# snayfach/MicrobeCensus

Hardware: AMD Instinct MI355X
Metric: reads/sec searched vs marker DB + AGS abs-error, 150 bp @ 1/2/4/8 GPU (higher is better)
Workload: dtype u8/int32

## Files before the change

microbecensus_amd/csrc/k_translate_seg.h:

```cpp
#pragma once
#include "mc_hip_common.h"

#define MC_TS_THREADS 64
#define MC_TS_WAVES (MC_TS_THREADS / 64)
#define MC_TS_READS (MC_TS_THREADS / 6)
#define MC_TS_NLNF(FP) ((FP) + 2 > 24 ? (FP) + 2 : 24)
#define MC_TS_STRIDE(FP) (((((FP) + 76 + 3) >> 2) | 1) << 2)
#define MC_TS_STAGE(L) ((((MC_TS_READS * (L)) > MC_TS_WAVES * 1488 ? (MC_TS_READS * (L)) : MC_TS_WAVES * 1488) + 15) & ~15)

struct McSegWaveLds { unsigned long long best[64]; uint32_t pre[66]; uint32_t pre2[66]; uint32_t bq[64]; uint16_t off[64]; uint8_t n[64]; };
static_assert(sizeof(McHsp) == 48 && sizeof(McGapTask) % 4 == 0, "k_eval_seeds copies its staging buffers as 16- and 4-byte words");
static_assert(sizeof(McSegWaveLds) == 1488, "MC_TS_STAGE reserves 1488 bytes per wave");
#ifdef MC_EXP_TIMING
__device__ unsigned long long g_ts_acc[12], g_ts_cnt[12];
#define MC_TS_TICK(k) do { const unsigned long long now_ = __builtin_readcyclecounter(); if (lane == 0) { ts_acc_[tcat_] += now_ - tlast_; ts_acc_[12 + tcat_] += 1; } tlast_ = now_; tcat_ = (k); } while (0)
#define MC_TS_BEGIN(k) __shared__ unsigned long long ts_acc_[24]; if (lane < 24) ts_acc_[lane] = 0; mc_wave_sync(); unsigned long long tlast_ = __builtin_readcyclecounter(); int tcat_ = (k)
#define MC_TS_PARAMS , unsigned long long &tlast_, int &tcat_, unsigned long long *ts_acc_
#define MC_TS_ARGS , tlast_, tcat_, ts_acc_
#define MC_TS_END do { mc_wave_sync(); if (lane < 12) { atomicAdd(&g_ts_acc[lane], ts_acc_[lane]); atomicAdd(&g_ts_cnt[lane], ts_acc_[12 + lane]); } } while (0)
#else
#define MC_TS_TICK(k) do { } while (0)
#define MC_TS_BEGIN(k) do { } while (0)
#define MC_TS_PARAMS
#define MC_TS_ARGS
#define MC_TS_END do { } while (0)
#endif
#define MC_SEG_KEY_ONE 0xBFF0000000000000ull

__device__ __forceinline__ unsigned long long mc_seg_key(double x)
{
    const unsigned long long u = (unsigned long long)__double_as_longlong(x);
    return (u >> 63) ? ~u : (u | 0x8000000000000000ull);
}

__device__ __forceinline__ void mc_seg_wave(const double *lnf, const int32_t *fx, const uint64_t *__restrict__ segtab, uint8_t *prot, int n, bool act, const McSegWS ws, McSegWaveLds *WL,
                                         const uint8_t *lds0, int lane MC_TS_PARAMS)
{
    const int W = (n <= 11) ? 8 : 12;
    MC_TS_TICK(0);
    enum { POP = 0, SCAN = 1, WAIT = 2, DONE = 3 };
    int st = (act && W <= n) ? POP : DONE;
    McBits192 Flo, Fhi, lo, nhi, mk;
    mc_bits_clear(Flo); mc_bits_clear(Fhi); mc_bits_clear(lo); mc_bits_clear(nhi); mc_bits_clear(mk);
    if (st != DONE) {
        mc_seg_window_flags_rg(fx, prot, n, W, Flo, Fhi);
        if (!(Flo.a | Flo.b | Flo.c)) st = DONE;
    }
    int sp = 1, base = 0, m = 0, i = 0, lowlim = 0, loi = 0, hii = 0;
    bool any = false;
    if (st != DONE) ws.stk[0] = (int16_t)(uint16_t)(n << 8);
    const unsigned long long ltmask = (1ull << lane) - 1;
    for (;;) {
        MC_TS_TICK(1);
        while (st == POP || st == SCAN) {
            if (st == POP) {
                if (sp == 0) { st = DONE; break; }
                sp--;
                base = MC_SEG_START(ws.stk[sp]); m = MC_SEG_LEN(ws.stk[sp]);
                if (W > m) continue;
                lo = mc_seg_flags_of(Flo, base, m, W);
                i = mc_bits_next(lo, 0);
                if (i >= m) continue;
                nhi = mc_bits_andnot(mc_bits_low(m), mc_seg_flags_of(Fhi, base, m, W));
                lowlim = 0; st = SCAN;
            }
            loi = mc_bits_prev(nhi, i) + 1; if (loi < lowlim) loi = lowlim;
            hii = mc_bits_next(nhi, i) - 1; if (hii > m - 1) hii = m - 1;
            st = WAIT;
        }
        const unsigned long long req = __ballot(st == WAIT);
        MC_TS_TICK(2);
        if (req == 0) break;
        const int nreq = __popcll(req);
        const int myr = __popcll(req & ltmask);
        const int myn = hii - loi + 1;
        if (st == WAIT) {
            WL->off[myr] = (uint16_t)((prot + base + loi) - lds0);
            WL->n[myr] = (uint8_t)myn;
            WL->best[myr] = MC_SEG_KEY_ONE; WL->bq[myr] = 0xFFFFFFFFu;
        }
        mc_wave_sync();
#define MC_SEG_CJ(j, sh) (((((j) >> (sh)) * (((j) >> (sh)) + 1)) << (sh)) / 2 + ((j) & ((1 << (sh)) - 1)) * (((j) >> (sh)) + 1))
        int sh0 = 3, sh1 = 3;
        {
            int K = 0, j0 = 0;
            if (lane < nreq) { const int nn = WL->n[lane], minlen = (nn - 100 > 1) ? nn - 100 : 1; K = nn - minlen; j0 = nn - 15 > 0 ? (nn - 15 < K ? nn - 15 : K) : 0; }
            uint32_t s0 = 0, s1 = 0;
#pragma unroll
            for (int sh = 2; sh >= 0; sh--) {
                const uint32_t c1 = (uint32_t)MC_SEG_CJ(j0, sh), c0 = (uint32_t)MC_SEG_CJ(K, sh) - c1;
                const uint32_t t0 = (uint32_t)__builtin_amdgcn_readlane((int)mc_wave_scan_add(c0), 63), t1 = (uint32_t)__builtin_amdgcn_readlane((int)mc_wave_scan_add(c1), 63);
                if (t0 <= 64) sh0 = sh;
                if (t1 <= 64) sh1 = sh;
            }
            {
                const uint32_t c1 = sh1 == 0 ? (uint32_t)MC_SEG_CJ(j0, 0) : sh1 == 1 ? (uint32_t)MC_SEG_CJ(j0, 1) : sh1 == 2 ? (uint32_t)MC_SEG_CJ(j0, 2) : (uint32_t)MC_SEG_CJ(j0, 3);
// ... 67 lines not shown
                        if (w0 == wlast) break;
                        mc_seg_shift(ws.comp, ws.sv, s[w0], s[w0 + len]);
                    }
                }
            }
            MC_TS_TICK(5);
            const bool cand = ok && key < MC_SEG_KEY_ONE;
            const unsigned long long old = WL->best[r];
            mc_wave_sync();
            if (cand) atomicMin(&WL->best[r], key);
            mc_wave_sync();
            const unsigned long long nb = WL->best[r];
            if (ok && nb != old) WL->bq[r] = 0xFFFFFFFFu;
            mc_wave_sync();
            if (cand && key == nb) atomicMin(&WL->bq[r], kq);
            mc_wave_sync();
        }
        }
#undef MC_SEG_CJ
        MC_TS_TICK(6);
        if (st == WAIT) {
            const uint32_t q = WL->bq[myr];
            int lend = 0, rend = myn - 1;
            if (q != 0xFFFFFFFFu) {
                int j = (int)((sqrtf((float)(8u * q + 1u)) - 1.0f) * 0.5f);
                while ((uint32_t)((j + 1) * (j + 2) / 2) <= q) j++;
                while ((uint32_t)(j * (j + 1) / 2) > q) j--;
                const int len = myn - j, w0 = (int)q - j * (j + 1) / 2;
                lend = w0; rend = len + w0 - 1;
            }
            const int leftend = loi + lend, rightend = hii - (myn - rend - 1);
            if (i < leftend) {
                const int l2 = loi, r2 = leftend - 1;
                sp = mc_seg_push(ws.stk, sp, W, base + l2, r2 - l2 + 1);
            }
            mk = mc_bits_or(mk, mc_bits_range(base + leftend, base + rightend));
            any = true;
            lowlim = ((hii < rightend) ? hii : rightend) + 1;
            i = mc_bits_next(lo, lowlim);
            st = i < m ? SCAN : POP;
        }
        mc_wave_sync();
    }
    MC_TS_TICK(7);
    if (any) for (int k = 0; k < n; k++) if (mc_bits_test(mk, k)) prot[k] = MC_INV;
    MC_TS_TICK(10);
}

__device__ __forceinline__ int mc_translate_frame_lds(const uint8_t *cod, const uint8_t *read, int len, int frame, uint8_t *prot)
{
    const int o = frame % 3;
    int n = (len - o) / 3;
    if (n < 0) n = 0;
    const bool rc = frame >= 3;
    const uint32_t set = rc ? MC_NT_RC_SET : MC_NT_FWD_SET, perm = rc ? MC_NT_RC_PERM : MC_NT_FWD_PERM;
    const uint8_t *p = read + (rc ? len - 1 - o : o);
    const int s = rc ? -1 : 1;
    int i = 0;
    for (; i + 8 <= n; i += 8) {
        uint32_t b[24], w[2] = {0, 0};
#pragma unroll
        for (int k = 0; k < 24; k++) b[k] = p[s * (3 * i + k)];
#pragma unroll
        for (int k = 0; k < 8; k++) {
            const int a0 = mc_nt_code(b[3 * k], set, perm), a1 = mc_nt_code(b[3 * k + 1], set, perm), a2 = mc_nt_code(b[3 * k + 2], set, perm);
            const uint32_t aa = cod[(16 * a0 + 4 * a1 + a2) & 63];
            w[k >> 2] |= ((a0 | a1 | a2) < 0 ? (uint32_t)MC_INV : aa) << (8 * (k & 3));
        }
        *(uint32_t *)(prot + i) = w[0];
        *(uint32_t *)(prot + i + 4) = w[1];
    }
    for (; i < n; i++) {
        const int a0 = mc_nt_code(p[s * (3 * i)], set, perm), a1 = mc_nt_code(p[s * (3 * i + 1)], set, perm), a2 = mc_nt_code(p[s * (3 * i + 2)], set, perm);
        const uint8_t aa = cod[(16 * a0 + 4 * a1 + a2) & 63];
        prot[i] = (a0 | a1 | a2) < 0 ? (uint8_t)MC_INV : aa;
    }
    return n;
}

template <bool STAGED>
__global__ void __attribute__((amdgpu_waves_per_eu(4, 4))) __launch_bounds__(MC_TS_THREADS) k_translate_seg(const McTables *__restrict__ T, const uint8_t *__restrict__ reads, int L,
                                                       int64_t nreads, uint8_t *__restrict__ frames, int FP, const uint64_t *__restrict__ segtab)
{
    extern __shared__ __attribute__((aligned(16))) uint8_t smem[];
    const int tid = threadIdx.x;
    const int64_t r0 = (int64_t)blockIdx.x * MC_TS_READS;
    const int nr = (int)((nreads - r0) < MC_TS_READS ? (nreads - r0) : MC_TS_READS);
    const int rbytes = nr * L;
    const int stride = MC_TS_STRIDE(FP);
    __shared__ int32_t fxs[64];
#ifdef MC_EXP_TIMING
    const int lane = mc_lane();
#endif
    MC_TS_BEGIN(8);
    uint8_t *sreads = smem;
    const int nlnf = MC_TS_NLNF(FP);
    double *lnf = (double *)(smem + (STAGED ? MC_TS_STAGE(L) : MC_TS_STAGE(0)));
    uint8_t *rows = (uint8_t *)(lnf + nlnf);
    __shared__ __attribute__((aligned(4))) uint8_t cod[64];
    if (tid < 64) fxs[tid] = T->seg_dout[tid];
    if (tid < 16) ((uint32_t *)cod)[tid] = ((const uint32_t *)T->codon)[tid];
    for (int i = tid; i < nlnf; i += MC_TS_THREADS) lnf[i] = T->lnfac[i];
    if (STAGED) {
        const uint8_t *src = reads + r0 * L;
        const int head = (int)((4 - ((uintptr_t)src & 3)) & 3), nhead = head < rbytes ? head : rbytes;
        if (tid < nhead) sreads[tid] = src[tid];
        const int nw = (rbytes - nhead) >> 2;
        if (nhead == 0) for (int i = tid; i < nw; i += MC_TS_THREADS) ((uint32_t *)sreads)[i] = ((const uint32_t *)src)[i];
        else for (int i = tid; i < nw; i += MC_TS_THREADS) { const uint32_t w = ((const uint32_t *)(src + nhead))[i]; uint8_t *d = sreads + nhead + 4 * i; d[0] = (uint8_t)w; d[1] = (uint8_t)(w >> 8); d[2] = (uint8_t)(w >> 16); d[3] = (uint8_t)(w >> 24); }
        for (int i = nhead + 4 * nw + tid; i < rbytes; i += MC_TS_THREADS) sreads[i] = src[i];
    }
    __syncthreads();
    MC_TS_TICK(9);
    const int lr = tid / 6, f = tid - lr * 6;
    uint8_t *prot = rows + (size_t)tid * stride;
    int n = 0;
    if (lr < nr) n = mc_translate_frame_lds(cod, STAGED ? sreads + lr * L : reads + (r0 + lr) * L, L, f, prot);
    __syncthreads();
    {
        McSegWS ws; ws.comp = prot + FP; ws.sv = prot + FP + 20; ws.stk = (int16_t *)(prot + FP + 44);
        mc_seg_wave(lnf, fxs, segtab, prot, n, lr < nr, ws, (McSegWaveLds *)smem + (tid >> 6), rows, mc_lane() MC_TS_ARGS);
        if (lr < nr) for (int i = n; i < FP; i++) prot[i] = MC_INV;
    }
    __syncthreads();
    {
        uint32_t *dst = (uint32_t *)(frames + r0 * 6 * FP);
        const int total = nr * 6 * FP / 4, fpw = FP / 4;
        for (int i = tid; i < total; i += MC_TS_THREADS) { const int row = i / fpw, col = i - row * fpw; dst[i] = *(const uint32_t *)(rows + (size_t)row * stride + 4 * col); }
    }
    MC_TS_TICK(0);
    MC_TS_END;
}
```

microbecensus_amd/csrc/mc_core.h:

```cpp
#pragma once
#include <stdint.h>

#if defined(__HIPCC__)
#include <hip/hip_runtime.h>
#define MC_HD __host__ __device__ __forceinline__
#define MC_HDN __host__ __device__
#else
#define MC_HD inline
#define MC_HDN inline
struct uint4 { uint32_t x, y, z, w; };
inline uint4 make_uint4(uint32_t x, uint32_t y, uint32_t z, uint32_t w) { uint4 v; v.x = x; v.y = y; v.z = z; v.w = w; return v; }
#endif

#define MC_NBUCKET 1000000
#define MC_INV 20
#define MC_INVGRP 10
#define MC_MAXAA 170
#define MC_SMAX 4096
#define MC_MAX_M8 500
#define MC_LNFAC_N 400

#define MC_GAP_OPEN 11
#define MC_GAP_EXT 1
#define MC_SEG_FXBITS 24
// ... 176 lines not shown
    }
    double ans2 = lnfac[total];
    for (int i = 0; sv[i] != 0; i++) ans2 = ans2 - lnfac[sv[i]];
    double t = (double)total * 2.995732273553991;
    return (ans2 + ans1) - t;
}
MC_HD void mc_seg_trim(const McTables &T, const uint8_t *s, int n, int *leftend, int *rightend)
{
    int lend = 0, rend = n - 1, minlen = 1;
    double minprob = 1.0;
    uint8_t comp[20], sv[21];
    if (n - 100 > minlen) minlen = n - 100;
    for (int len = n; len > minlen; len--) {
        mc_seg_comp(s, len, comp);
        for (int i = 0;; i++) {
            mc_seg_state(comp, sv);
            double prob = mc_seg_getprob(T.lnfac, sv, len);
            if (prob < minprob) { minprob = prob; lend = i; rend = len + i - 1; }
            if (i + 1 + len > n) break;
            if (s[i] < 20) comp[s[i]]--;
            if (s[i + len] < 20) comp[s[i + len]]++;
        }
    }
    *leftend = *leftend + lend;
    *rightend = *rightend - (n - rend - 1);
}
#define MC_SEG_STK 16
static_assert(MC_MAXAA / 13 < MC_SEG_STK && MC_MAXAA <= 255, "the SEG work list: n / (W + 1) entries of 8 + 8 bits");
#ifndef MC_SEG_ON_FULL
#define MC_SEG_ON_FULL() ((void)0)
#endif
#define MC_SEG_START(e) ((int)((uint16_t)(e) & 255))
#define MC_SEG_LEN(e) ((int)((uint16_t)(e) >> 8))
MC_HD int mc_seg_push(int16_t *stk, int sp, int W, int start, int len)
{
    if (len < W) return sp;
    if (sp >= MC_SEG_STK) { MC_SEG_ON_FULL(); return sp; }
    stk[sp] = (int16_t)(uint16_t)(start | (len << 8));
    return sp + 1;
}
MC_HDN void mc_seg_mask(const McTables &T, const uint8_t *prot, int n, uint8_t *maskbits , double *H)
{
    int W = (n <= 11) ? 8 : 12;
    int16_t stk[MC_SEG_STK];
    int sp = 0;
    for (int i = 0; i < (MC_MAXAA + 7) / 8; i++) maskbits[i] = 0;
    stk[0] = (int16_t)(uint16_t)(n << 8); sp = 1;
    while (sp > 0) {
        sp--;
        int base = MC_SEG_START(stk[sp]), m = MC_SEG_LEN(stk[sp]);
        const uint8_t *s = prot + base;
        if (W > m) continue;
        {
            uint8_t comp[20], sv[21];
            int start = 0;
            mc_seg_comp(s, W, comp);
            mc_seg_state(comp, sv);
            double ent = mc_seg_entropy(T, W, sv);
            for (int i = 0; i <= m - 1; i++) {
                H[i] = ent;
                if (start + 1 + W <= m) {
                    if (s[start] < 20) comp[s[start]]--;
                    if (s[start + W] < 20) comp[s[start + W]]++;
                    start++;
                    mc_seg_state(comp, sv);
                    ent = mc_seg_entropy(T, W, sv);
                }
            }
        }
        int last = m - 1, lowlim = 0;
        for (int i = 0; i <= last; i++) {
            if (H[i] <= 2.2 && H[i] != -1.0) {
                int j, loi, hii, leftend, rightend;
// ... 143 lines not shown
    uint32_t x = (lo ^ (hi << 7) ^ (((hi >> 28) * 0x924000u) & 0x04444000u)) * 0xBA1BF32Fu;
    x ^= x >> 15;
    h1 = x >> (32 - MC_SEGTAB_LOG2);
    h2 = (x >> 6) & (MC_SEGTAB_SLOTS - 1);
}
MC_HD uint64_t mc_segtab_lookup(const uint64_t *tab, uint64_t hist, int len)
{
    const uint64_t k = hist | ((uint64_t)len << 60);
    uint32_t h1, h2;
    mc_segtab_slots(k, h1, h2);
    if (tab[2 * h1] == k) return tab[2 * h1 + 1];
    return tab[2 * h2] == k ? tab[2 * h2 + 1] : 0;
}

MC_HD void mc_seg_trim_rg(const double *lnfac, const uint8_t *s, int n, int *leftend, int *rightend)
{
    int lend = 0, rend = n - 1;
    double minprob = 1.0;
    McRgState st0; st0.clo = 0; st0.chi = 0; st0.sv = 0;
    for (int k = 0; k < n; k++) mc_rg_add(st0, s[k]);
    for (int len = n; len > 1; len--) {
        McRgState st = st0;
        for (int i = 0;; i++) {
            const double prob = mc_rg_getprob(lnfac, st.sv, len);
            if (prob < minprob) { minprob = prob; lend = i; rend = len + i - 1; }
            if (i + 1 + len > n) break;
            mc_rg_remove(st, s[i]); mc_rg_add(st, s[i + len]);
        }
        mc_rg_remove(st0, s[len - 1]);
    }
    *leftend = *leftend + lend;
    *rightend = *rightend - (n - rend - 1);
}
struct McBits192 { uint64_t a, b, c; };
MC_HD void mc_bits_clear(McBits192 &x) { x.a = 0; x.b = 0; x.c = 0; }
MC_HD void mc_bits_set(McBits192 &x, int i) { uint64_t m = 1ull << (i & 63); if (i < 64) x.a |= m; else if (i < 128) x.b |= m; else x.c |= m; }
MC_HD bool mc_bits_test(const McBits192 &x, int i) { uint64_t w = (i < 64) ? x.a : (i < 128) ? x.b : x.c; return (w >> (i & 63)) & 1; }

MC_HDN void mc_seg_mask_ws(const McTables &T, uint8_t *prot, int n, const McSegWS &ws)
{
    int W = (n <= 11) ? 8 : 12;
    McBits192 lo, hi, mk;
    mc_bits_clear(mk);
    if (W > n) return;
    int sp = 1;
    ws.stk[0] = (int16_t)(uint16_t)(n << 8);
    bool any = false;
    while (sp > 0) {
        sp--;
        int base = MC_SEG_START(ws.stk[sp]), m = MC_SEG_LEN(ws.stk[sp]);
        const uint8_t *s = prot + base;
        if (W > m) continue;
        mc_bits_clear(lo); mc_bits_clear(hi);
        {
            int start = 0;
            bool anylo = false;
            mc_seg_comp(s, W, ws.comp);
            mc_seg_state(ws.comp, ws.sv);
            double ent = mc_seg_entropy(T, W, ws.sv);
            for (int i = 0; i <= m - 1; i++) {
                if (ent <= 2.2) { mc_bits_set(lo, i); anylo = true; }
                if (ent <= 2.5) mc_bits_set(hi, i);
                if (start + 1 + W <= m) {
                    mc_seg_shift(ws.comp, ws.sv, s[start], s[start + W]);
                    start++;
                    ent = mc_seg_entropy(T, W, ws.sv);
                }
            }
            if (!anylo) continue;
        }
// ... 91 lines not shown
    else { r.a = w0; r.b = w1; r.c = w2; }
    return r;
}
MC_HD McBits192 mc_bits_low(int n)
{
    McBits192 r;
    r.a = n >= 64 ? ~0ull : (n > 0 ? (1ull << n) - 1 : 0);
    r.b = n >= 128 ? ~0ull : (n > 64 ? (1ull << (n - 64)) - 1 : 0);
    r.c = n >= 192 ? ~0ull : (n > 128 ? (1ull << (n - 128)) - 1 : 0);
    return r;
}
MC_HD McBits192 mc_bits_and(const McBits192 &x, const McBits192 &y) { McBits192 r; r.a = x.a & y.a; r.b = x.b & y.b; r.c = x.c & y.c; return r; }
MC_HD McBits192 mc_bits_or(const McBits192 &x, const McBits192 &y) { McBits192 r; r.a = x.a | y.a; r.b = x.b | y.b; r.c = x.c | y.c; return r; }
MC_HD McBits192 mc_bits_andnot(const McBits192 &x, const McBits192 &y) { McBits192 r; r.a = x.a & ~y.a; r.b = x.b & ~y.b; r.c = x.c & ~y.c; return r; }
MC_HD McBits192 mc_bits_range(int lo, int hi) { return mc_bits_andnot(mc_bits_low(hi + 1), mc_bits_low(lo)); }
MC_HD int mc_bits_next(const McBits192 &x, int from)
{
    if (from >= 192) return 192;
    McBits192 y = mc_bits_andnot(x, mc_bits_low(from));
    if (y.a) return __builtin_ctzll(y.a);
    if (y.b) return 64 + __builtin_ctzll(y.b);
    if (y.c) return 128 + __builtin_ctzll(y.c);
    return 192;
}
MC_HD int mc_bits_prev(const McBits192 &x, int from)
{
    if (from < 0) return -1;
    McBits192 y = mc_bits_and(x, mc_bits_low(from + 1));
    if (y.c) return 191 - __builtin_clzll(y.c);
    if (y.b) return 127 - __builtin_clzll(y.b);
    if (y.a) return 63 - __builtin_clzll(y.a);
    return -1;
}
MC_HD McBits192 mc_seg_flags_of(const McBits192 &F, int base, int m, int W)
{
    McBits192 r = mc_bits_and(mc_bits_shr(F, base), mc_bits_low(m - W + 1));
    if (mc_bits_test(r, m - W)) r = mc_bits_or(r, mc_bits_range(m - W + 1, m - 1));
    return r;
}
MC_HD void mc_seg_window_flags(const int32_t *fx, const uint8_t *s, int n, int W, uint8_t *comp, McBits192 &Flo, McBits192 &Fhi)
{
    mc_bits_clear(Flo); mc_bits_clear(Fhi);
    int S = 0, t = 0;
    for (int i = 0; i < 20; i++) comp[i] = 0;
    for (int i = 0; i < W; i++) { const int r = s[i]; if (r < 20) { const int c = comp[r]; S += fx[16 + c]; comp[r] = (uint8_t)(c + 1); t++; } }
    for (int x = 0;; x++) {
        if (S >= fx[32 + t]) mc_bits_set(Flo, x);
        if (S >= fx[48 + t]) mc_bits_set(Fhi, x);
        if (x + 1 + W > n) break;
        const int o = s[x], e = s[x + W];
        if (o < 20) { const int c = comp[o]; S += fx[c]; comp[o] = (uint8_t)(c - 1); t--; }
        if (e < 20) { const int c = comp[e]; S += fx[16 + c]; comp[e] = (uint8_t)(c + 1); t++; }
    }
}
MC_HD void mc_seg_window_flags_rg(const int32_t *fx, const uint8_t *s, int n, int W, McBits192 &Flo, McBits192 &Fhi)
{
    uint64_t clo = 0; uint32_t chi = 0;
    int S = 0, t = 0;
    for (int i = 0; i < W; i++) {
        const int r = s[i];
        if (r < 20) {
            const int sh = (r & 15) * 4;
            const int c = (r < 16) ? (int)((clo >> sh) & 15) : (int)((chi >> sh) & 15);
            S += fx[16 + c]; t++;
            if (r < 16) clo += 1ull << sh; else chi += 1u << sh;
        }
    }
    const int nwin = n - W + 1;
    uint64_t wl[3] = {0, 0, 0}, wh[3] = {0, 0, 0};
#if defined(__HIP_DEVICE_COMPILE__)
#pragma unroll
#endif
    for (int q = 0; q < 3; q++) {
        uint64_t a = 0, b = 0;
        const int x1 = nwin - 64 * q < 64 ? nwin - 64 * q : 64;
        for (int xx = 0; xx < x1; xx++) {
            const int x = 64 * q + xx;
            a |= (uint64_t)(S >= fx[32 + t]) << xx;
            b |= (uint64_t)(S >= fx[48 + t]) << xx;
            if (x + 1 < nwin) {
                const int o = s[x], e = s[x + W];
                if (o < 20) {
                    const int sh = (o & 15) * 4;
                    const int c = (o < 16) ? (int)((clo >> sh) & 15) : (int)((chi >> sh) & 15);
                    S += fx[c]; t--;
                    if (o < 16) clo -= 1ull << sh; else chi -= 1u << sh;
                }
                if (e < 20) {
                    const int sh = (e & 15) * 4;
                    const int c = (e < 16) ? (int)((clo >> sh) & 15) : (int)((chi >> sh) & 15);
                    S += fx[16 + c]; t++;
                    if (e < 16) clo += 1ull << sh; else chi += 1u << sh;
                }
            }
        }
        wl[q] = a; wh[q] = b;
    }
    Flo.a = wl[0]; Flo.b = wl[1]; Flo.c = wl[2];
    Fhi.a = wh[0]; Fhi.b = wh[1]; Fhi.c = wh[2];
}
MC_HDN void mc_seg_mask_fx2(const double *lnfac, const int32_t *fx, uint8_t *prot, int n, const McSegWS &ws)
{
    const int W = (n <= 11) ? 8 : 12;
    if (W > n) return;
    McBits192 Flo, Fhi, mk;
    mc_bits_clear(mk);
    mc_seg_window_flags(fx, prot, n, W, ws.comp, Flo, Fhi);
    if (!(Flo.a | Flo.b | Flo.c)) return;
    int sp = 1;
    ws.stk[0] = (int16_t)(uint16_t)(n << 8);
    bool any = false;
    while (sp > 0) {
        sp--;
        const int base = MC_SEG_START(ws.stk[sp]), m = MC_SEG_LEN(ws.stk[sp]);
        const uint8_t *s = prot + base;
        if (W > m) continue;
        const McBits192 lo = mc_seg_flags_of(Flo, base, m, W), hi = mc_seg_flags_of(Fhi, base, m, W);
        const McBits192 nhi = mc_bits_andnot(mc_bits_low(m), hi);
        int lowlim = 0;
        for (int i = mc_bits_next(lo, 0); i < m; i = mc_bits_next(lo, i + 1)) {
            int loi = mc_bits_prev(nhi, i) + 1; if (loi < lowlim) loi = lowlim;
            int hii = mc_bits_next(nhi, i) - 1; if (hii > m - 1) hii = m - 1;
            int leftend = loi, rightend = hii;
            if (rightend - leftend + 1 <= 15) mc_seg_trim_rg(lnfac, s + leftend, rightend - leftend + 1, &leftend, &rightend);
            else mc_seg_trim_ws(lnfac, s + leftend, rightend - leftend + 1, &leftend, &rightend, ws);
            if (i < leftend) {
                const int lend = loi, rend = leftend - 1;
                sp = mc_seg_push(ws.stk, sp, W, base + lend, rend - lend + 1);
            }
            mk = mc_bits_or(mk, mc_bits_range(base + leftend, base + rightend));
            any = true;
            i = (hii < rightend) ? hii : rightend;
            lowlim = i + 1;
        }
    }
    if (any) for (int i = 0; i < n; i++) if (mc_bits_test(mk, i)) prot[i] = MC_INV;
}

MC_HD int mc_klen(uint32_t k)
{
    int low = (k & 0xf) != 0xf;
    int l = ((k & 0xff) != 0xff) ? 3 + low : 2 + low;
    l -= ((k & 0xfff) == 0xfff);
    l -= (k == 0xffff);
    return l;
}
MC_HD bool mc_key_lb_less(uint32_t dbk, uint32_t qk)
{
    int ld = mc_klen(dbk), lq = mc_klen(qk), n = ld < lq ? ld : lq;
    if (n != 0) { int sh = (4 - n) * 4; int a = (int)(dbk >> sh), b = (int)(qk >> sh); if (a != b) return a < b; }
    return ld < lq;
}
MC_HD bool mc_key_ub_less(uint32_t qk, uint32_t dbk)
{
    int ld = mc_klen(dbk), lq = mc_klen(qk), n = lq <= ld ? lq : ld;
    if (n == 0) return lq < ld;
    int sh = (4 - n) * 4; int a = (int)(qk >> sh), b = (int)(dbk >> sh);
    if (a == b) return false;
    return a < b;
}
struct McSeedCount { uint32_t lookups, keyprobes, tasks; };

MC_HD int mc_key_range(const McIndex &X, int seed, uint32_t qk, int *nst_out, McSeedCount *sc)
// ... 658 lines not shown
```

microbecensus_amd/csrc/mc_hip.hip:

```cpp
#include "mc_hip_common.h"
#include "k_translate_seg.h"
#include "k_enumerate.h"
#include "k_eval_seeds.h"
#include "k_gapped.h"
#include "k_order.h"
#include "k_finish.h"
#include "mc_stages.h"
#include "k_grid.h"
#include "k_simulate.h"
#include "k_community.h"
#include "k_varlen.h"
#include "k_classes.h"
#include "k_bootstrap.h"
#include "k_wfit.h"
#include "mc_pieces.h"
#include "mc_ahead.h"
#include "mc_owned.h"
#include "mc_abund.h"

#include <map>

struct McCtx {
    McStream stream; hipStream_t side = nullptr, side2 = nullptr;
    McEvent ev[8], ev_fork, ev_join, ev_join2;
    McEvent ev_wait[2]; bool waited = false;
    int64_t cap_reads = 0; int pool_len = 0;
    int ts_staged = -1;
    uint32_t cap_tasks = 0, cap_gaps = 0, cap_hsps = 0, cap_rows = 0;
    McDev<uint8_t> d_frames_base[2]; uint8_t *d_frames = nullptr;
    uint8_t *frames_of(int b) const { return d_frames_base[b] + 64; }
    void frames_use(int b) { d_frames = frames_of(b); }
    McDev<unsigned long long> d_stats;
    McDev<McSeedTask> d_tasks; McDev<McGapTask> d_gaps; McDev<McHsp> d_hsps, d_v, d_tmp;
    McDev<uint64_t> d_k64, d_hkeys, d_hplace, d_places; McDev<uint32_t> d_idx, d_idxo, d_heads, d_scan, d_gsz, d_nv, d_ghist;
    McDev<uint32_t> d_counters;
    McDev<McRow> d_rows; McDev<uint32_t> d_nrow, d_rowoff; McDev<McBestHit> d_best, d_bestof; McDev<uint8_t> d_low, d_cand;
    McDev<McGapCell> d_gws_full; McDev<uint32_t> d_retry, d_retry2;
    McDev<unsigned long long> d_gtab; uint32_t gtab_slots = 0; McDev<uint32_t> d_gleader; McDev<McFlankOut> d_fout;
    McPin<uint32_t> h_c; McPin<unsigned long long> h_stats; McPin<McBestHit> h_best; size_t h_best_cap = 0;
    const uint8_t *reads = nullptr; int64_t n = 0, first_read_id = 0, first = 0;
    int ahead_from = -1;
    bool predicts = false;
    bool own_a0 = true;
    uint32_t ntasks = 0, ngaps = 0, gpad = 0, nh = 0, nh_all = 0, nheads = 0, nrows = 0, nbest = 0, nsegs = 0;
    bool busy = false;
};

struct mc_handle {
    McHostIndex H;
    std::vector<int32_t> fam;
    int nfam = 0, device = 0;
    McDev<uint8_t> d_res_base; uint8_t *d_res = nullptr; McDev<uint32_t> d_off, d_bstart, d_post; McDev<unsigned long long> d_post8; McDev<uint16_t> d_keys; McDev<int32_t> d_fam;
    McDev<McTables> d_T; McDev<McClassPars> d_P;
    McTables hT; McClassPars hP;
    int read_len = 0, FP = 0; bool run_set = false;
    McDev<uint32_t> d_bitmap;
    McDev<McBucketRec> d_rec;
    McDev<uint32_t> d_filt, d_wild, d_pair; McDev<uint64_t> d_segtab; McDev<unsigned long long> d_rt;
    bool fast_enum = false;
    bool count_traffic = false;
// ... 456 lines not shown
            for (int k = 0; k < 7; k++) fprintf(stderr, "ev-timing %-21s total %9.1f Mcycles (lane 0 of every wave)\n", en[k], ev[k] / 1e6);
            unsigned long long z8[8] = {0, 0, 0, 0, 0, 0, 0, 0};
            HIPCK(hipMemcpyToSymbol(HIP_SYMBOL(g_ev_acc), z8, sizeof z8));
            unsigned long long tr[4];
            HIPCK(hipMemcpyFromSymbol(tr, HIP_SYMBOL(g_ev_turns), sizeof tr));
            fprintf(stderr, "ev-turns forward: %.1f M lane-turns in %.2f M wave-turns = %.1f lanes of 64; backward: %.1f M in %.2f M = %.1f lanes\n", tr[0] / 1e6, tr[1] / 1e6, tr[1] ? (double)tr[0] / (double)tr[1] : 0.0,
                    tr[2] / 1e6, tr[3] / 1e6, tr[3] ? (double)tr[2] / (double)tr[3] : 0.0);
            HIPCK(hipMemcpyToSymbol(HIP_SYMBOL(g_ev_turns), z8, sizeof tr));
        }
        const char *nm[8] = {"group starts", "groups", "scan, items", "sort", "threshold, ranks", "heap sort", "rows", "other"};
        for (int k = 0; k < 8; k++) fprintf(stderr, "fh-timing %-17s total %9.1f Mcycles %9llu entries\n", nm[k], acc[k] / 1e6, cnt[k]);
        {
            unsigned long long w[12];
            HIPCK(hipMemcpyFromSymbol(w, HIP_SYMBOL(g_fh_worst), sizeof w));
            fprintf(stderr, "fh-worst read: %llu stacked HSPs, %.3f Mcycles:", w[0] & 0xFFFFF, (double)(w[0] >> 20) / 1e6);
            for (int k = 0; k < 8; k++) fprintf(stderr, " %s %.3f", nm[k], (double)w[1 + k] / 1e6);
            fprintf(stderr, "\n");
            unsigned long long z12[12] = {0, 0, 0, 0, 0, 0, 0, 0, 0, 0, 0, 0};
            HIPCK(hipMemcpyToSymbol(HIP_SYMBOL(g_fh_worst), z12, sizeof z12));
        }
        unsigned long long z[8] = {0, 0, 0, 0, 0, 0, 0, 0};
        HIPCK(hipMemcpyToSymbol(HIP_SYMBOL(g_fh_acc), z, sizeof z)); HIPCK(hipMemcpyToSymbol(HIP_SYMBOL(g_fh_cnt), z, sizeof z));
    }
    return 0;
}
#else
static int exp_timing_dump(mc_handle *, McCtx &, char) { return 0; }
#endif

static int stage_a0(mc_handle *h, McCtx &c, hipStream_t st, const uint8_t *reads, uint8_t *into, int64_t at, int64_t n, hipEvent_t e0, hipEvent_t e1)
{
    uint8_t *frames = into + at * 6 * h->FP;
    HIPCK(hipEventRecord(e0, st));
    if (mc_translate_launch(h->d_T, h->d_segtab, reads, h->read_len, h->FP, n, frames, st, &c.ts_staged)) return -1;
    HIPCK(hipEventRecord(e1, st));
    return 0;
}

static int stage_a(mc_handle *h, McCtx &c, int64_t covered)
{
    const int64_t n = c.n;
    hipStream_t st = c.stream;
    c.ntasks = c.ngaps = c.gpad = c.nh = c.nheads = c.nrows = c.nbest = c.nsegs = 0;
    HIPCK(hipMemsetAsync(c.d_counters, 0, sizeof(uint32_t) * C_N, st));
    HIPCK(hipMemsetAsync(c.d_stats, 0, sizeof(unsigned long long) * S_N, st));
    if (h->best_only) HIPCK(hipMemsetAsync(c.d_cand, 0, (size_t)n, st));
    HIPCK(hipMemsetAsync(c.d_low, 0, (size_t)n, st));
    c.own_a0 = covered < n;
    if (!c.own_a0) HIPCK(hipEventRecord(c.ev[1], st));
    else if (stage_a0(h, c, st, c.reads + covered * h->read_len, c.d_frames, covered, n - covered, c.ev[0], c.ev[1])) return -1;
    if (exp_timing_dump(h, c, 'a')) return -1;
    const McRun R = run_of(h);
    const McSeedBufs B = carve_seed(h, c);
    const McSeedKernel kind = !h->fast_enum ? MC_SEED_PLAIN : h->count_traffic ? MC_SEED_COUNTING : MC_SEED_QUEUES;
    if (mc_enumerate_launch(R, B, n, kind, st)) return -1;
    HIPCK(hipEventRecord(c.ev[2], st));
    if (mc_eval_seeds_launch(R, B, kind == MC_SEED_QUEUES, st)) return -1;
    HIPCK(hipEventRecord(c.ev[3], st));
    return counters_to_host(c);
}

static int stage_b(mc_handle *h, McCtx &c)
{
    hipStream_t st = c.stream;
    if (c.h_c[C_OVERFLOW]) { g_err = "seed task / HSP / gap task buffer overflow"; return -2; }
    c.ntasks = c.h_c[C_TASKS];
    const uint32_t ngaps = c.ngaps = c.h_c[C_GAPS];
// ... 213 lines not shown
    return range_end(h, c);
}

static int range_begin_checked(mc_handle *h, int64_t first, int64_t count, int64_t first_read_id, bool predicts)
{
    if (range_check(h, first, count)) return -1;
    if (count <= 0) { g_err = "mc_range_begin: an empty range"; return -1; }
    if (h->pipe_nout) { g_err = "mc_range_begin: a range is in flight already (mc_range_end first)"; return -1; }
    const int rc = range_begin(h, h->ctx, first, count, first_read_id, predicts);
    if (rc) return rc;
    h->pipe_nout = 1;
    return 0;
}
extern "C" int mc_range_begin(mc_handle *h, int64_t first, int64_t count, int64_t first_read_id) { return range_begin_checked(h, first, count, first_read_id, true); }

static int range_end_next(mc_handle *h, int64_t first, int64_t count) { return range_end(h, h->ctx, first, count); }

extern "C" int64_t mc_ranges_translated_ahead(const mc_handle *h) { return h ? h->ahead_used : 0; }
extern "C" float mc_ahead_kernel_ms(const mc_handle *h) { return h ? h->ahead_ms : 0.0f; }

extern "C" int mc_range_end(mc_handle *h)
{
    if (!h) { g_err = "null handle"; return -1; }
    if (h->pipe_nout == 0) { g_err = "mc_range_end: no range in flight"; return -1; }
    HIPCK(hipSetDevice(h->device));
    h->pipe_nout = 0;
    return range_end(h, h->ctx);
}

extern "C" int mc_ranges_in_flight(const mc_handle *h) { return h ? h->pipe_nout : 0; }

extern "C" int64_t mc_debug_stage(mc_handle *h, int what, void *dst, int64_t cap_bytes, int32_t *record_bytes)
{
    if (!h || !h->run_set || what < 0 || what > 5) { g_err = "mc_debug_stage: bad argument"; return -1; }
    if (h->pipe_nout) { g_err = "mc_debug_stage: ranges are in flight"; return -1; }
    HIPCK(hipSetDevice(h->device));
    ahead_drop(h);
    const McCtx &c = h->ctx;
    if (what == 4) {
        if (!c.h_c) { g_err = "mc_debug_stage: no range has run"; return -1; }
        const uint32_t v[3] = {c.h_c[C_ITEMS], c.h_c[C_RETRY], c.h_c[C_RETRY2]};
        if (record_bytes) *record_bytes = (int32_t)sizeof(uint32_t);
        if (dst && (int64_t)sizeof v <= cap_bytes) memcpy(dst, v, sizeof v);
        return (int64_t)sizeof v;
    }
    if (what == 5) {
        if (c.ts_staged < 0) { g_err = "mc_debug_stage: no range has run"; return -1; }
        const uint32_t v = (uint32_t)c.ts_staged;
        if (record_bytes) *record_bytes = (int32_t)sizeof v;
        if (dst && (int64_t)sizeof v <= cap_bytes) memcpy(dst, &v, sizeof v);
        return (int64_t)sizeof v;
    }
    const void *src = nullptr; int64_t bytes = 0; int32_t rec = 0;
    if (what == 0) { src = c.d_frames; rec = h->FP; bytes = c.n * 6 * (int64_t)h->FP; }
    else if (what == 1) { src = c.d_tasks; rec = (int32_t)sizeof(McSeedTask); bytes = (int64_t)c.ntasks * rec; }
    else if (what == 2) { src = c.d_gaps; rec = (int32_t)sizeof(McGapTask); bytes = (int64_t)c.ngaps * rec; }
    else { src = c.d_hsps; rec = (int32_t)sizeof(McHsp); bytes = (int64_t)(c.nh_all + (c.h_c ? c.h_c[C_HPAD] : 0u)) * rec; }
    if (record_bytes) *record_bytes = rec;
    if (dst && bytes && bytes <= cap_bytes) { HIPCK(hipStreamSynchronize(c.stream)); HIPCK(hipMemcpy(dst, src, (size_t)bytes, hipMemcpyDeviceToHost)); }
    return bytes;
}

extern "C" int mc_set_counting(mc_handle *h, int on)
{
    if (!h) { g_err = "null handle"; return -1; }
    ahead_drop(h);
    h->count_traffic = on != 0;
    return 0;
}

extern "C" int mc_run(mc_handle *h, int64_t first_read_id) { return h ? mc_run_range(h, 0, h->nreads, first_read_id) : -1; }

#define MC_STREAM_BATCH 2000000
static int64_t stream_batch()
{
    if (const char *e = getenv("MC_STREAM_BATCH")) { const long long v = atoll(e); if (v >= 1000 && v <= MC_STREAM_BATCH) return (int64_t)v; }
    return MC_STREAM_BATCH;
}
struct McBatchSlot { uint8_t *pin = nullptr, *dev = nullptr; int64_t n = 0, first = 0; int state = 0;  int64_t rc = 0; };

static int run_stream(mc_handle *h, const std::function<int64_t(uint8_t *, int64_t, int64_t *)> &fetch, int64_t first_read_id, int64_t expect_reads = 0)
// ... 1659 lines not shown
```

microbecensus_amd/csrc/mc_stages.h:

```cpp
#pragma once
#include "k_translate_seg.h"
#include "k_enumerate.h"
#include "k_eval_seeds.h"
#include "k_gapped.h"
#include "k_order.h"
#include "k_finish.h"

static constexpr uint32_t MC_CUS = 256u;
static constexpr int MC_GAP_THREADS_FULL = 16 * 1024;
static constexpr uint32_t MC_GAP_SORT_BLOCKS = 512u;
static constexpr uint32_t MC_GAP_GRID_MAX = MC_CUS * 8u;
static constexpr uint32_t MC_GAP_GRID2 = MC_CUS * 4u;
static constexpr uint32_t MC_GAP_GRID_FULL = (uint32_t)MC_GAP_THREADS_FULL / 128u;
static constexpr uint32_t MC_BIN_BLOCKS = MC_CUS * 8u;
static inline size_t mc_order_heavy_lds(uint32_t cap) { return (size_t)cap * 18; }
static inline size_t mc_finish_heavy_lds(int maxn) { return (size_t)maxn * 16 + 3 * (size_t)(maxn + 2) * 2; }
static inline size_t mc_heap_lanes_lds() { return (size_t)(MC_MAX_M8 + 2) * 64 * 4; }
static inline size_t mc_finish_lds(int tpb, int items) { return (size_t)tpb * (items * 16 + 16); }

struct McRun { const McTables *T; McIndex X; const McClassPars *P; const int32_t *fam; int L, FP; };
struct McFork { hipStream_t side, side2; hipEvent_t fork, join, join2; };

static int mc_translate_launch(const McTables *T, const uint64_t *segtab, const uint8_t *reads, int L, int FP, int64_t n, uint8_t *frames, hipStream_t st, int *staged_out = nullptr)
{
    const size_t lds_rest = (size_t)MC_TS_NLNF(FP) * 8 + (size_t)MC_TS_THREADS * MC_TS_STRIDE(FP);
    const size_t lds_staged = (size_t)MC_TS_STAGE(L) + lds_rest, lds_direct = (size_t)MC_TS_STAGE(0) + lds_rest;
    static const int ts_force = getenv("MC_TS_STAGED") ? atoi(getenv("MC_TS_STAGED")) : -1;
    const size_t cu_lds = 160 * 1024 - 1024;
    const bool staged = ts_force >= 0 ? ts_force != 0 : cu_lds / lds_staged >= cu_lds / lds_direct;
    const size_t lds = staged ? lds_staged : lds_direct;
    if (staged_out) *staged_out = staged ? 1 : 0;
    const unsigned ts_blocks = (unsigned)((n + MC_TS_READS - 1) / MC_TS_READS);
    if (staged) {
        if (lds > 48 * 1024) HIPCK(hipFuncSetAttribute((const void *)k_translate_seg<true>, hipFuncAttributeMaxDynamicSharedMemorySize, (int)lds));
        k_translate_seg<true><<<dim3(ts_blocks), dim3(MC_TS_THREADS), lds, st>>>(T, reads, L, n, frames, FP, segtab);
    } else {
        if (lds > 48 * 1024) HIPCK(hipFuncSetAttribute((const void *)k_translate_seg<false>, hipFuncAttributeMaxDynamicSharedMemorySize, (int)lds));
        k_translate_seg<false><<<dim3(ts_blocks), dim3(MC_TS_THREADS), lds, st>>>(T, reads, L, n, frames, FP, segtab);
    }
    return 0;
}

struct McSeedBufs {
    const uint8_t *frames; const uint32_t *bitmap; McSeedTask *tasks; uint32_t cap_tasks; uint32_t *counters; unsigned long long *stats;
    McHsp *hsps; uint32_t cap_hsps; McGapTask *gaps; uint32_t cap_gaps; uint8_t *cand; uint64_t *hkeys; uint8_t *low; uint64_t *hplace;
};
enum McSeedKernel { MC_SEED_PLAIN, MC_SEED_QUEUES, MC_SEED_COUNTING };

static int mc_enumerate_launch(const McRun &R, const McSeedBufs &B, int64_t n, McSeedKernel kind, hipStream_t st)
{
    const int L = R.L, FP = R.FP;
    if (kind != MC_SEED_PLAIN) {
        const bool enq = kind == MC_SEED_QUEUES;
        const size_t per_wave = enq ? MC_ENQ_WAVE_LDS(FP, L) : sizeof(McEnWave) + MC_EN_WAVE_LDS(FP, L);
        int waves = 0, bpc = 1;
        {
            static const int shapes_q[][2] = {{8, 2}, {4, 4}, {16, 1}, {12, 1}, {4, 3}, {8, 1}, {4, 2}, {4, 1}};
            static const int shapes_c[][2] = {{12, 2}, {8, 3}, {4, 6}, {4, 5}, {16, 1}, {8, 2}, {4, 4}, {12, 1}, {4, 3}, {8, 1}, {4, 2}, {4, 1}};
            if (enq) { for (const auto &sh : shapes_q) if (!waves && (size_t)sh[1] * (64 + sh[0] * per_wave) <= 160 * 1024) { waves = sh[0]; bpc = sh[1]; } }
            else for (const auto &sh : shapes_c) if (!waves && (size_t)sh[1] * (64 + sh[0] * per_wave) <= 160 * 1024) { waves = sh[0]; bpc = sh[1]; }
        }
        if (!waves) { g_err = "reads too long for the seed kernel's LDS layout"; return -1; }
        const size_t lds2 = 64 + waves * per_wave;
#define MC_LAUNCH_EN(KERNEL, WV)                                                                                                                   \
    do {                                                                                                                                           \
        HIPCK(hipFuncSetAttribute((const void *)KERNEL<WV>, hipFuncAttributeMaxDynamicSharedMemorySize, (int)lds2));                               \
// ... 167 lines not shown
```

Before: 69.80 million.

## Add narrow 64-bit SEG bitset kernel variant for short reads

Templates the SEG low-complexity masking on the bitset type and adds a narrow k_translate_seg variant that uses a single 64-bit word and a four-entry work stack whenever the translated length fits in 63 residues, which holds for 150 bp reads. The narrow variant shrinks per-thread LDS rows and gives the 4 idle threads a small spare area instead of full rows. It raises the waves-per-EU hint from 4 to 5. The aim is fewer registers and less LDS per block so more waves fit per CU, at the cost of an extra kernel instantiation and a capped work stack.

```diff
diff --git a/microbecensus_amd/csrc/k_translate_seg.h b/microbecensus_amd/csrc/k_translate_seg.h
--- a/microbecensus_amd/csrc/k_translate_seg.h
+++ b/microbecensus_amd/csrc/k_translate_seg.h
@@ -6,6 +6,9 @@
 #define MC_TS_READS (MC_TS_THREADS / 6)
 #define MC_TS_NLNF(FP) ((FP) + 2 > 24 ? (FP) + 2 : 24)
 #define MC_TS_STRIDE(FP) (((((FP) + 76 + 3) >> 2) | 1) << 2)
+#define MC_TS_STRIDE_N(FP) (((((FP) + 44 + 2 * MC_SEG_STK_NARROW + 3) >> 2) | 1) << 2)
+#define MC_TS_SPARE 48
+#define MC_TS_ROWS_N(FP) ((size_t)(6 * MC_TS_READS) * MC_TS_STRIDE_N(FP) + (size_t)(MC_TS_THREADS - 6 * MC_TS_READS) * MC_TS_SPARE)
 #define MC_TS_STAGE(L) ((((MC_TS_READS * (L)) > MC_TS_WAVES * 1488 ? (MC_TS_READS * (L)) : MC_TS_WAVES * 1488) + 15) & ~15)
 
 struct McSegWaveLds { unsigned long long best[64]; uint32_t pre[66]; uint32_t pre2[66]; uint32_t bq[64]; uint16_t off[64]; uint8_t n[64]; };
@@ -33,6 +36,7 @@
     return (u >> 63) ? ~u : (u | 0x8000000000000000ull);
 }
 
+template <class BS>
 __device__ __forceinline__ void mc_seg_wave(const double *lnf, const int32_t *fx, const uint64_t *__restrict__ segtab, uint8_t *prot, int n, bool act, const McSegWS ws, McSegWaveLds *WL,
                                          const uint8_t *lds0, int lane MC_TS_PARAMS)
 {
@@ -40,11 +44,11 @@
     MC_TS_TICK(0);
     enum { POP = 0, SCAN = 1, WAIT = 2, DONE = 3 };
     int st = (act && W <= n) ? POP : DONE;
-    McBits192 Flo, Fhi, lo, nhi, mk;
+    BS Flo, Fhi, lo, nhi, mk;
     mc_bits_clear(Flo); mc_bits_clear(Fhi); mc_bits_clear(lo); mc_bits_clear(nhi); mc_bits_clear(mk);
     if (st != DONE) {
         mc_seg_window_flags_rg(fx, prot, n, W, Flo, Fhi);
-        if (!(Flo.a | Flo.b | Flo.c)) st = DONE;
+        if (!mc_bits_any(Flo)) st = DONE;
     }
     int sp = 1, base = 0, m = 0, i = 0, lowlim = 0, loi = 0, hii = 0;
     bool any = false;
@@ -61,7 +65,7 @@
                 lo = mc_seg_flags_of(Flo, base, m, W);
                 i = mc_bits_next(lo, 0);
                 if (i >= m) continue;
-                nhi = mc_bits_andnot(mc_bits_low(m), mc_seg_flags_of(Fhi, base, m, W));
+                nhi = mc_bits_andnot(mc_bits_low(mk, m), mc_seg_flags_of(Fhi, base, m, W));
                 lowlim = 0; st = SCAN;
             }
             loi = mc_bits_prev(nhi, i) + 1; if (loi < lowlim) loi = lowlim;
@@ -195,9 +199,9 @@
             const int leftend = loi + lend, rightend = hii - (myn - rend - 1);
             if (i < leftend) {
                 const int l2 = loi, r2 = leftend - 1;
-                sp = mc_seg_push(ws.stk, sp, W, base + l2, r2 - l2 + 1);
-            }
-            mk = mc_bits_or(mk, mc_bits_range(base + leftend, base + rightend));
+                sp = mc_seg_push_cap(ws.stk, sp, W, base + l2, r2 - l2 + 1, BS::STK);
+            }
+            mk = mc_bits_or(mk, mc_bits_range(mk, base + leftend, base + rightend));
             any = true;
             lowlim = ((hii < rightend) ? hii : rightend) + 1;
             i = mc_bits_next(lo, lowlim);
@@ -241,8 +245,10 @@
     return n;
 }
 
-template <bool STAGED>
-__global__ void __attribute__((amdgpu_waves_per_eu(4, 4))) __launch_bounds__(MC_TS_THREADS) k_translate_seg(const McTables *__restrict__ T, const uint8_t *__restrict__ reads, int L,
+template <bool NARROW> struct McTsBits { typedef McBits192 T; };
+template <> struct McTsBits<true> { typedef McBits64 T; };
+template <bool STAGED, bool NARROW = false>
+__global__ void __attribute__((amdgpu_waves_per_eu(NARROW ? 5 : 4, NARROW ? 5 : 4))) __launch_bounds__(MC_TS_THREADS) k_translate_seg(const McTables *__restrict__ T, const uint8_t *__restrict__ reads, int L,
                                                        int64_t nreads, uint8_t *__restrict__ frames, int FP, const uint64_t *__restrict__ segtab)
 {
     extern __shared__ __attribute__((aligned(16))) uint8_t smem[];
@@ -250,7 +256,7 @@
     const int64_t r0 = (int64_t)blockIdx.x * MC_TS_READS;
     const int nr = (int)((nreads - r0) < MC_TS_READS ? (nreads - r0) : MC_TS_READS);
     const int rbytes = nr * L;
-    const int stride = MC_TS_STRIDE(FP);
+    const int stride = NARROW ? MC_TS_STRIDE_N(FP) : MC_TS_STRIDE(FP);
     __shared__ int32_t fxs[64];
 #ifdef MC_EXP_TIMING
     const int lane = mc_lane();
@@ -277,12 +283,14 @@
     MC_TS_TICK(9);
     const int lr = tid / 6, f = tid - lr * 6;
     uint8_t *prot = rows + (size_t)tid * stride;
+    uint8_t *wsp = prot + FP;
+    if (NARROW && tid >= 6 * MC_TS_READS) { prot = rows; wsp = rows + (size_t)(6 * MC_TS_READS) * stride + (size_t)(tid - 6 * MC_TS_READS) * MC_TS_SPARE; }
     int n = 0;
     if (lr < nr) n = mc_translate_frame_lds(cod, STAGED ? sreads + lr * L : reads + (r0 + lr) * L, L, f, prot);
     __syncthreads();
     {
-        McSegWS ws; ws.comp = prot + FP; ws.sv = prot + FP + 20; ws.stk = (int16_t *)(prot + FP + 44);
-        mc_seg_wave(lnf, fxs, segtab, prot, n, lr < nr, ws, (McSegWaveLds *)smem + (tid >> 6), rows, mc_lane() MC_TS_ARGS);
+        McSegWS ws; ws.comp = wsp; ws.sv = wsp + 20; ws.stk = (int16_t *)(wsp + 44);
+        mc_seg_wave<typename McTsBits<NARROW>::T>(lnf, fxs, segtab, prot, n, lr < nr, ws, (McSegWaveLds *)smem + (tid >> 6), rows, mc_lane() MC_TS_ARGS);
         if (lr < nr) for (int i = n; i < FP; i++) prot[i] = MC_INV;
     }
     __syncthreads();
diff --git a/microbecensus_amd/csrc/mc_core.h b/microbecensus_amd/csrc/mc_core.h
--- a/microbecensus_amd/csrc/mc_core.h
+++ b/microbecensus_amd/csrc/mc_core.h
@@ -232,13 +232,17 @@
 #endif
 #define MC_SEG_START(e) ((int)((uint16_t)(e) & 255))
 #define MC_SEG_LEN(e) ((int)((uint16_t)(e) >> 8))
-MC_HD int mc_seg_push(int16_t *stk, int sp, int W, int start, int len)
+MC_HD int mc_seg_push_cap(int16_t *stk, int sp, int W, int start, int len, int cap)
 {
     if (len < W) return sp;
-    if (sp >= MC_SEG_STK) { MC_SEG_ON_FULL(); return sp; }
+    if (sp >= cap) { MC_SEG_ON_FULL(); return sp; }
     stk[sp] = (int16_t)(uint16_t)(start | (len << 8));
     return sp + 1;
 }
+MC_HD int mc_seg_push(int16_t *stk, int sp, int W, int start, int len) { return mc_seg_push_cap(stk, sp, W, start, len, MC_SEG_STK); }
+#define MC_NARROW_MAXAA 63
+#define MC_SEG_STK_NARROW 4
+static_assert(MC_NARROW_MAXAA / 13 <= MC_SEG_STK_NARROW && MC_NARROW_MAXAA < 64, "the narrow SEG work list; no shift by 64 in McBits64");
 MC_HDN void mc_seg_mask(const McTables &T, const uint8_t *prot, int n, uint8_t *maskbits , double *H)
 {
     int W = (n <= 11) ? 8 : 12;
@@ -448,10 +452,18 @@
     *leftend = *leftend + lend;
     *rightend = *rightend - (n - rend - 1);
 }
-struct McBits192 { uint64_t a, b, c; };
+struct McBits192 { uint64_t a, b, c; static constexpr int WORDS = 3, STK = MC_SEG_STK; };
 MC_HD void mc_bits_clear(McBits192 &x) { x.a = 0; x.b = 0; x.c = 0; }
 MC_HD void mc_bits_set(McBits192 &x, int i) { uint64_t m = 1ull << (i & 63); if (i < 64) x.a |= m; else if (i < 128) x.b |= m; else x.c |= m; }
 MC_HD bool mc_bits_test(const McBits192 &x, int i) { uint64_t w = (i < 64) ? x.a : (i < 128) ? x.b : x.c; return (w >> (i & 63)) & 1; }
+MC_HD bool mc_bits_any(const McBits192 &x) { return (x.a | x.b | x.c) != 0; }
+MC_HD void mc_bits_from_words(McBits192 &x, const uint64_t *w) { x.a = w[0]; x.b = w[1]; x.c = w[2]; }
+struct McBits64 { uint64_t a; static constexpr int WORDS = 1, STK = MC_SEG_STK_NARROW; };
+MC_HD void mc_bits_clear(McBits64 &x) { x.a = 0; }
+MC_HD void mc_bits_set(McBits64 &x, int i) { x.a |= 1ull << i; }
+MC_HD bool mc_bits_test(const McBits64 &x, int i) { return (x.a >> i) & 1; }
+MC_HD bool mc_bits_any(const McBits64 &x) { return x.a != 0; }
+MC_HD void mc_bits_from_words(McBits64 &x, const uint64_t *w) { x.a = w[0]; }
 
 MC_HDN void mc_seg_mask_ws(const McTables &T, uint8_t *prot, int n, const McSegWS &ws)
 {
@@ -609,13 +621,35 @@
     if (y.a) return 63 - __builtin_clzll(y.a);
     return -1;
 }
-MC_HD McBits192 mc_seg_flags_of(const McBits192 &F, int base, int m, int W)
-{
-    McBits192 r = mc_bits_and(mc_bits_shr(F, base), mc_bits_low(m - W + 1));
-    if (mc_bits_test(r, m - W)) r = mc_bits_or(r, mc_bits_range(m - W + 1, m - 1));
+MC_HD McBits64 mc_bits_shr(const McBits64 &x, int k) { McBits64 r; r.a = x.a >> k; return r; }
+MC_HD McBits64 mc_bits_low(const McBits64 &, int n) { McBits64 r; r.a = (1ull << n) - 1; return r; }
+MC_HD McBits192 mc_bits_low(const McBits192 &, int n) { return mc_bits_low(n); }
+MC_HD McBits64 mc_bits_and(const McBits64 &x, const McBits64 &y) { McBits64 r; r.a = x.a & y.a; return r; }
+MC_HD McBits64 mc_bits_or(const McBits64 &x, const McBits64 &y) { McBits64 r; r.a = x.a | y.a; return r; }
+MC_HD McBits64 mc_bits_andnot(const McBits64 &x, const McBits64 &y) { McBits64 r; r.a = x.a & ~y.a; return r; }
+MC_HD McBits64 mc_bits_range(const McBits64 &t, int lo, int hi) { return mc_bits_andnot(mc_bits_low(t, hi + 1), mc_bits_low(t, lo)); }
+MC_HD McBits192 mc_bits_range(const McBits192 &, int lo, int hi) { return mc_bits_range(lo, hi); }
+MC_HD int mc_bits_next(const McBits64 &x, int from)
+{
+    if (from >= 64) return 64;
+    const uint64_t y = x.a & (~0ull << from);
+    return y ? __builtin_ctzll(y) : 64;
+}
+MC_HD int mc_bits_prev(const McBits64 &x, int from)
+{
+    if (from < 0) return -1;
+    const uint64_t y = x.a & ((2ull << from) - 1);
+    return y ? 63 - __builtin_clzll(y) : -1;
+}
+template <class B>
+MC_HD B mc_seg_flags_of(const B &F, int base, int m, int W)
+{
+    B r = mc_bits_and(mc_bits_shr(F, base), mc_bits_low(F, m - W + 1));
+    if (mc_bits_test(r, m - W)) r = mc_bits_or(r, mc_bits_range(F, m - W + 1, m - 1));
     return r;
 }
-MC_HD void mc_seg_window_flags(const int32_t *fx, const uint8_t *s, int n, int W, uint8_t *comp, McBits192 &Flo, McBits192 &Fhi)
+template <class B>
+MC_HD void mc_seg_window_flags(const int32_t *fx, const uint8_t *s, int n, int W, uint8_t *comp, B &Flo, B &Fhi)
 {
     mc_bits_clear(Flo); mc_bits_clear(Fhi);
     int S = 0, t = 0;
@@ -630,7 +664,8 @@
         if (e < 20) { const int c = comp[e]; S += fx[16 + c]; comp[e] = (uint8_t)(c + 1); t++; }
     }
 }
-MC_HD void mc_seg_window_flags_rg(const int32_t *fx, const uint8_t *s, int n, int W, McBits192 &Flo, McBits192 &Fhi)
+template <class B>
+MC_HD void mc_seg_window_flags_rg(const int32_t *fx, const uint8_t *s, int n, int W, B &Flo, B &Fhi)
 {
     uint64_t clo = 0; uint32_t chi = 0;
     int S = 0, t = 0;
@@ -648,7 +683,7 @@
 #if defined(__HIP_DEVICE_COMPILE__)
 #pragma unroll
 #endif
-    for (int q = 0; q < 3; q++) {
+    for (int q = 0; q < B::WORDS; q++) {
         uint64_t a = 0, b = 0;
         const int x1 = nwin - 64 * q < 64 ? nwin - 64 * q : 64;
         for (int xx = 0; xx < x1; xx++) {
@@ -673,17 +708,18 @@
         }
         wl[q] = a; wh[q] = b;
     }
-    Flo.a = wl[0]; Flo.b = wl[1]; Flo.c = wl[2];
-    Fhi.a = wh[0]; Fhi.b = wh[1]; Fhi.c = wh[2];
-}
+    mc_bits_from_words(Flo, wl);
+    mc_bits_from_words(Fhi, wh);
+}
+template <class B = McBits192>
 MC_HDN void mc_seg_mask_fx2(const double *lnfac, const int32_t *fx, uint8_t *prot, int n, const McSegWS &ws)
 {
     const int W = (n <= 11) ? 8 : 12;
     if (W > n) return;
-    McBits192 Flo, Fhi, mk;
+    B Flo, Fhi, mk;
     mc_bits_clear(mk);
     mc_seg_window_flags(fx, prot, n, W, ws.comp, Flo, Fhi);
-    if (!(Flo.a | Flo.b | Flo.c)) return;
+    if (!mc_bits_any(Flo)) return;
     int sp = 1;
     ws.stk[0] = (int16_t)(uint16_t)(n << 8);
     bool any = false;
@@ -692,8 +728,8 @@
         const int base = MC_SEG_START(ws.stk[sp]), m = MC_SEG_LEN(ws.stk[sp]);
         const uint8_t *s = prot + base;
         if (W > m) continue;
-        const McBits192 lo = mc_seg_flags_of(Flo, base, m, W), hi = mc_seg_flags_of(Fhi, base, m, W);
-        const McBits192 nhi = mc_bits_andnot(mc_bits_low(m), hi);
+        const B lo = mc_seg_flags_of(Flo, base, m, W), hi = mc_seg_flags_of(Fhi, base, m, W);
+        const B nhi = mc_bits_andnot(mc_bits_low(mk, m), hi);
         int lowlim = 0;
         for (int i = mc_bits_next(lo, 0); i < m; i = mc_bits_next(lo, i + 1)) {
             int loi = mc_bits_prev(nhi, i) + 1; if (loi < lowlim) loi = lowlim;
@@ -703,9 +739,9 @@
             else mc_seg_trim_ws(lnfac, s + leftend, rightend - leftend + 1, &leftend, &rightend, ws);
             if (i < leftend) {
                 const int lend = loi, rend = leftend - 1;
-                sp = mc_seg_push(ws.stk, sp, W, base + lend, rend - lend + 1);
-            }
-            mk = mc_bits_or(mk, mc_bits_range(base + leftend, base + rightend));
+                sp = mc_seg_push_cap(ws.stk, sp, W, base + lend, rend - lend + 1, B::STK);
+            }
+            mk = mc_bits_or(mk, mc_bits_range(mk, base + leftend, base + rightend));
             any = true;
             i = (hii < rightend) ? hii : rightend;
             lowlim = i + 1;
diff --git a/microbecensus_amd/csrc/mc_hip.hip b/microbecensus_amd/csrc/mc_hip.hip
--- a/microbecensus_amd/csrc/mc_hip.hip
+++ b/microbecensus_amd/csrc/mc_hip.hip
@@ -26,6 +26,7 @@
     McEvent ev_wait[2]; bool waited = false;
     int64_t cap_reads = 0; int pool_len = 0;
     int ts_staged = -1;
+    int ts_narrow = -1;
     uint32_t cap_tasks = 0, cap_gaps = 0, cap_hsps = 0, cap_rows = 0;
     McDev<uint8_t> d_frames_base[2]; uint8_t *d_frames = nullptr;
     uint8_t *frames_of(int b) const { return d_frames_base[b] + 64; }
@@ -548,7 +549,7 @@
 {
     uint8_t *frames = into + at * 6 * h->FP;
     HIPCK(hipEventRecord(e0, st));
-    if (mc_translate_launch(h->d_T, h->d_segtab, reads, h->read_len, h->FP, n, frames, st, &c.ts_staged)) return -1;
+    if (mc_translate_launch(h->d_T, h->d_segtab, reads, h->read_len, h->FP, n, frames, st, &c.ts_staged, &c.ts_narrow)) return -1;
     HIPCK(hipEventRecord(e1, st));
     return 0;
 }
@@ -828,7 +829,7 @@
 
 extern "C" int64_t mc_debug_stage(mc_handle *h, int what, void *dst, int64_t cap_bytes, int32_t *record_bytes)
 {
-    if (!h || !h->run_set || what < 0 || what > 5) { g_err = "mc_debug_stage: bad argument"; return -1; }
+    if (!h || !h->run_set || what < 0 || what > 6) { g_err = "mc_debug_stage: bad argument"; return -1; }
     if (h->pipe_nout) { g_err = "mc_debug_stage: ranges are in flight"; return -1; }
     HIPCK(hipSetDevice(h->device));
     ahead_drop(h);
@@ -840,9 +841,9 @@
         if (dst && (int64_t)sizeof v <= cap_bytes) memcpy(dst, v, sizeof v);
         return (int64_t)sizeof v;
     }
-    if (what == 5) {
-        if (c.ts_staged < 0) { g_err = "mc_debug_stage: no range has run"; return -1; }
-        const uint32_t v = (uint32_t)c.ts_staged;
+    if (what == 5 || what == 6) {
+        if (c.ts_staged < 0 || c.ts_narrow < 0) { g_err = "mc_debug_stage: no range has run"; return -1; }
+        const uint32_t v = (uint32_t)(what == 5 ? c.ts_staged : c.ts_narrow);
         if (record_bytes) *record_bytes = (int32_t)sizeof v;
         if (dst && (int64_t)sizeof v <= cap_bytes) memcpy(dst, &v, sizeof v);
         return (int64_t)sizeof v;
diff --git a/microbecensus_amd/csrc/mc_stages.h b/microbecensus_amd/csrc/mc_stages.h
--- a/microbecensus_amd/csrc/mc_stages.h
+++ b/microbecensus_amd/csrc/mc_stages.h
@@ -21,7 +21,8 @@
 struct McRun { const McTables *T; McIndex X; const McClassPars *P; const int32_t *fam; int L, FP; };
 struct McFork { hipStream_t side, side2; hipEvent_t fork, join, join2; };
 
-static int mc_translate_launch(const McTables *T, const uint64_t *segtab, const uint8_t *reads, int L, int FP, int64_t n, uint8_t *frames, hipStream_t st, int *staged_out = nullptr)
+static int mc_translate_launch(const McTables *T, const uint64_t *segtab, const uint8_t *reads, int L, int FP, int64_t n, uint8_t *frames, hipStream_t st, int *staged_out = nullptr,
+                               int *narrow_out = nullptr)
 {
     const size_t lds_rest = (size_t)MC_TS_NLNF(FP) * 8 + (size_t)MC_TS_THREADS * MC_TS_STRIDE(FP);
     const size_t lds_staged = (size_t)MC_TS_STAGE(L) + lds_rest, lds_direct = (size_t)MC_TS_STAGE(0) + lds_rest;
@@ -31,7 +32,14 @@
     const size_t lds = staged ? lds_staged : lds_direct;
     if (staged_out) *staged_out = staged ? 1 : 0;
     const unsigned ts_blocks = (unsigned)((n + MC_TS_READS - 1) / MC_TS_READS);
-    if (staged) {
+    const bool narrow = L / 3 <= MC_NARROW_MAXAA;
+    static_assert(MC_NARROW_MAXAA <= 63 && MC_SEG_STK_NARROW * 13 + 12 >= MC_NARROW_MAXAA, "the narrow form's one-word bit sets and four-entry work list");
+    if (narrow_out) *narrow_out = narrow ? 1 : 0;
+    if (narrow) {
+        const size_t lds_n = (size_t)MC_TS_STAGE(staged ? L : 0) + (size_t)MC_TS_NLNF(FP) * 8 + MC_TS_ROWS_N(FP);
+        if (staged) k_translate_seg<true, true><<<dim3(ts_blocks), dim3(MC_TS_THREADS), lds_n, st>>>(T, reads, L, n, frames, FP, segtab);
+        else k_translate_seg<false, true><<<dim3(ts_blocks), dim3(MC_TS_THREADS), lds_n, st>>>(T, reads, L, n, frames, FP, segtab);
+    } else if (staged) {
         if (lds > 48 * 1024) HIPCK(hipFuncSetAttribute((const void *)k_translate_seg<true>, hipFuncAttributeMaxDynamicSharedMemorySize, (int)lds));
         k_translate_seg<true><<<dim3(ts_blocks), dim3(MC_TS_THREADS), lds, st>>>(T, reads, L, n, frames, FP, segtab);
     } else {
```

Measured after the change: 72.69 million, median of 6. 4.1% higher.
